# SysCV/sam-pt

Measured on AMD Instinct MI355X. Metric: frames/sec end-to-end (ViT-H + PIPS, 480p, 8 pts, 1 obj) at 1/2/4/8 MI355X, higher is better.
Workload: dtype f16; 1 GPU; SAM vit_h + PIPS, 8 query points, 1 object(s), 24x 480p synthetic frames upscaled to 576x1024, 12 refinement iterations, random-init weights (seed 72); submit=sequential: one blocking SamPt.forward per step, parallelism=sequence-sharded x1, decoder_precision=fp32

## Files before the change

sam_pt_amd/csrc/attention.hip:

```cpp
#include "ops.h"

namespace sampt {

typedef float f32x2 __attribute__((ext_vector_type(2)));

template <typename TQ>
__global__ __launch_bounds__(256) void k_vit_rel_bias(const TQ* __restrict__ qkv, const float* __restrict__ rel_h,
                                                      const float* __restrict__ rel_w, int S, int heads, int hd,
                                                      float* __restrict__ relhT, float* __restrict__ relwT) {
  extern __shared__ float qs[];
  const int qh = blockIdx.x, h = blockIdx.y, b = blockIdx.z;
  const int N = S * S, D = heads * hd, ldq = hd + 1;
  for (int i = threadIdx.x; i < S * hd; i += 256) {
    int t = i / hd, c = i - t * hd;
    qs[t * ldq + c] = (float)qkv[((long)(b * N + qh * S + t)) * 3 * D + h * hd + c];
  }
  __syncthreads();
  const long bh = (long)b * heads + h;
  for (int i = threadIdx.x; i < S * 2 * S; i += 256) {
    int kk = i / S, qw = i - kk * S;
    const float* tab;
    if (kk < S) tab = rel_h + (long)(qh - kk + S - 1) * hd;
    else tab = rel_w + (long)(qw - (kk - S) + S - 1) * hd;
    const float* qv = qs + qw * ldq;
    float a = 0.f;
    for (int c = 0; c < hd; ++c) a += qv[c] * tab[c];
    int q = qh * S + qw;
    if (kk < S) relhT[(bh * S + kk) * N + q] = a;
    else relwT[(bh * S + (kk - S)) * N + q] = a;
  }
}

int vit_rel_bias(const void* qkv, int qkv_f16, const float* rel_h, const float* rel_w, int B, int S, int heads,
                 int hd, float* relh, float* relw, hipStream_t s) {
  dim3 grid(S, heads, B), block(256);
  size_t sh = (size_t)S * (hd + 1) * sizeof(float);
  if (qkv_f16)
    hipLaunchKernelGGL(k_vit_rel_bias<half_t>, grid, block, sh, s, (const half_t*)qkv, rel_h, rel_w, S, heads, hd, relh,
                       relw);
  else
    hipLaunchKernelGGL(k_vit_rel_bias<float>, grid, block, sh, s, (const float*)qkv, rel_h, rel_w, S, heads, hd, relh,
                       relw);
  SAMPT_CHECK_LAUNCH("vit_rel_bias");
  return SAMPT_OK;
}

__global__ __launch_bounds__(256) void k_softmax_rel_rows(float* __restrict__ scores, const float* __restrict__ relhT,
                                                          const float* __restrict__ relwT, int N, int S) {
  __shared__ float red[8];
  const int q = blockIdx.x;
  const long bh = blockIdx.y;
  float* row = scores + (bh * N + q) * N;
  const float* rh = relhT + bh * S * N + q;
  const float* rw = relwT + bh * S * N + q;
  const int tid = threadIdx.x, lane = tid & 63, wave = tid >> 6;
  float m = -INFINITY;
  for (int k = tid; k < N; k += 256) {
    float v = row[k] + rh[(long)(k / S) * N] + rw[(long)(k % S) * N];
    row[k] = v;
    m = fmaxf(m, v);
  }
  m = wave_max(m);
  if (lane == 0) red[wave] = m;
  __syncthreads();
  m = fmaxf(fmaxf(red[0], red[1]), fmaxf(red[2], red[3]));
  float sum = 0.f;
  for (int k = tid; k < N; k += 256) {
    float e = expf(row[k] - m);
    row[k] = e;
    sum += e;
  }
  sum = wave_sum(sum);
  if (lane == 0) red[4 + wave] = sum;
  __syncthreads();
  sum = (red[4] + red[5]) + (red[6] + red[7]);
  for (int k = tid; k < N; k += 256) row[k] = row[k] / sum;
}

int softmax_rel_rows(float* scores, const float* relh, const float* relw, long BH, int Nq, int S, hipStream_t s) {
  if (Nq != S * S) return SAMPT_ERR_ARG;
  hipLaunchKernelGGL(k_softmax_rel_rows, dim3(Nq, (unsigned)BH), dim3(256), 0, s, scores, relh, relw, Nq, S);
  SAMPT_CHECK_LAUNCH("softmax_rel_rows");
  return SAMPT_OK;
}

__device__ half_t g_flash_pad[16] = {(half_t)1.f, (half_t)0.f, (half_t)0.f, (half_t)0.f, (half_t)0.f, (half_t)0.f,
                                     (half_t)0.f, (half_t)0.f, (half_t)0.f, (half_t)0.f, (half_t)0.f, (half_t)0.f,
                                     (half_t)0.f, (half_t)0.f, (half_t)0.f, (half_t)0.f};

template <int HD, int NW, int SG>
__global__ __launch_bounds__(NW * 64, NW == 4 ? 3 : 2) void k_flash_f16(const half_t* __restrict__ qkv, const float* __restrict__ rel_h,
                                                       const float* __restrict__ rel_w, half_t* __restrict__ out, int N,
                                                       int heads, float scale, FlashPad pad, int B, int uh) {
  constexpr int KS = HD / 16;
  constexpr int DT = (HD + 31) / 32;
  constexpr int QT = NW * 32;
  constexpr int NT = NW * 64;
  constexpr bool LROW = DT * 32 > HD;
  constexpr int VP = LROW ? DT * 32 : HD;
  constexpr int RLD = QT + 2;
  constexpr int CPR = HD / 8, CPV = VP / 8;
  constexpr int KSWZ = CPR == 8 ? 7 : (CPR == 4 ? 3 : (CPR == 10 ? 1 : 0)), KSH = CPR == 4 ? 2 : (CPR == 10 ? 3 : 1);
  constexpr int KB = 64 * HD * 2, VB = 64 * VP * 2, RELB = SG * RLD * 2;
  constexpr int BUFB = KB + VB > RELB ? KB + VB : ((RELB + 1023) / 1024) * 1024;
  __shared__ __attribute__((aligned(1024))) char tile_s[BUFB];
  __shared__ half_t relh_s[SG][RLD];
  half_t(*Ks)[64][HD] = (half_t(*)[64][HD])tile_s;
  half_t(*Vs)[64][VP] = (half_t(*)[64][VP])(tile_s + KB);
  half_t(*relw_s)[RLD] = (half_t(*)[RLD])tile_s;
  constexpr int NKI = (CPR + NW - 1) / NW, NVI = (CPV + NW - 1) / NW;
  __shared__ unsigned dma_tab[NKI + NVI][NT];

  const int tid = threadIdx.x, lane = tid & 63, wave = __builtin_amdgcn_readfirstlane(tid >> 6);
  const int li = lane & 31, hi = lane >> 5;
  int bx, h, b;
  flash_wg_decode(blockIdx.x, (N + QT - 1) / QT, heads, B, uh, bx, h, b);
  const int D = heads * HD;
  const long tok0 = (long)b * N;
  const int qblk = bx * QT;
  const int ql = wave * 32 + li;
  const int q = qblk + ql;
  const bool wave_live = qblk + wave * 32 < N;
  constexpr int RPT = SG >= 64 ? 1 : 64 / SG, KTV = SG >= 64 ? 64 : RPT * SG;
  constexpr float LOG2E = 1.4426950408889634f;
  const float c2 = scale * LOG2E;
  const int pw = pad.bias_row ? b % pad.nwin : 0;
  const int pwy = pw / max(pad.nwx, 1), py0 = pwy * SG, px0 = (pw - pwy * max(pad.nwx, 1)) * SG;
  auto is_pad = [&](int t) {
    const int iy = t / SG, ix = t - iy * SG;
    return pad.bias_row != nullptr && (py0 + iy >= pad.gh || px0 + ix >= pad.gw);
  };
  {
    int n = 0;
    for (int i = wave; i < CPR; i += NW, ++n) {
      const int e = i * 64 + lane, slot = e / CPR, c = e - slot * CPR;
      const int sc = min(slot, KTV - 1), siy = sc / SG, six = sc - siy * SG;
      const unsigned off = (unsigned)((c ^ ((slot >> KSH) & KSWZ)) * 16);
      dma_tab[n][tid] = (unsigned)sc | (unsigned)siy << 8 | (pad.bias_row != nullptr && px0 + six >= pad.gw ? 1u << 12 : 0u) | off << 16;
    }
    n = NKI;
    for (int i = wave; i < CPV; i += NW, ++n) {
      const int e = i * 64 + lane, slot = e / CPV, c = e - slot * CPV;
      const int sc = min(slot, KTV - 1), siy = sc / SG, six = sc - siy * SG;
      const int cs = HD == 64 ? c ^ (((slot >> 1) & 1) << 2) : c;
      const unsigned off = (unsigned)(c < CPR ? cs * 16 : (c - CPR) * 16);
      dma_tab[n][tid] = (unsigned)sc | (unsigned)siy << 8 | (pad.bias_row != nullptr && px0 + six >= pad.gw ? 1u << 12 : 0u) |
                        (c < CPR ? 0u : 1u << 13) | off << 16;
    }
  }
  auto dma_tile = [&](int kt0, int kh0, int buf) {
    const half_t* kbase = qkv + tok0 * 3 * D + D + h * HD;
    const unsigned stride = 3u * (unsigned)D * 2u;
    const char* kb = (const char*)kbase;
    const char* vb = (const char*)(kbase + D);
    const char* pk = (const char*)(pad.bias_row ? pad.bias_row + D + h * HD : kbase);
    const char* pv = (const char*)(pad.bias_row ? pad.bias_row + 2 * D + h * HD : kbase);
    int n = 0;
    for (int i = wave; i < CPR; i += NW, ++n) {
      const unsigned t = dma_tab[n][tid];
      const unsigned krow = min((unsigned)kt0 + (t & 255u), (unsigned)(N - 1));
      const int gr = kh0 + (int)(t >> 8 & 15u);
      const bool pd = pad.bias_row != nullptr && ((t & 0x1000u) != 0 || gr >= SG || py0 + gr >= pad.gh);
      const char* src = pd ? pk + (t >> 16) : kb + (__umul24(krow, stride) + (t >> 16));
      __builtin_amdgcn_global_load_lds((const __attribute__((address_space(1))) void*)src,
                                       (__attribute__((address_space(3))) void*)((char*)&Ks[buf][0][0] + i * 1024), 16, 0, 0);
    }
    n = NKI;
    for (int i = wave; i < CPV; i += NW, ++n) {
      const unsigned t = dma_tab[n][tid];
      const unsigned vrow = min((unsigned)kt0 + (t & 255u), (unsigned)(N - 1));
      const int gr = kh0 + (int)(t >> 8 & 15u);
      const bool pd = pad.bias_row != nullptr && ((t & 0x1000u) != 0 || gr >= SG || py0 + gr >= pad.gh);
      const char* src = pd ? pv + (t >> 16) : vb + (__umul24(vrow, stride) + (t >> 16));
      if (LROW && (t & 0x2000u)) src = (const char*)g_flash_pad + (t >> 16);
      __builtin_amdgcn_global_load_lds((const __attribute__((address_space(1))) void*)src,
                                       (__attribute__((address_space(3))) void*)((char*)&Vs[buf][0][0] + i * 1024), 16, 0, 0);
    }
  };

  for (int i = tid; i < SG * RLD; i += NT) {
    (&relh_s[0][0])[i] = (half_t)0.f;
    (&relw_s[0][0])[i] = (half_t)0.f;
  }
  h8 qf[KS];
#pragma unroll
  for (int ks = 0; ks < KS; ++ks) {
    if (q < N && !is_pad(q)) qf[ks] = *(const h8*)(qkv + (tok0 + q) * 3 * D + h * HD + ks * 16 + hi * 8);
    else qf[ks] = (h8){0, 0, 0, 0, 0, 0, 0, 0};
  }
  __syncthreads();
  {
    constexpr int NR = 2 * SG - 1, NTIL = (NR + 31) / 32;
    const int qh = q / SG, qw = q - qh * SG;
#pragma unroll
    for (int tb = 0; tb < 2; ++tb) {
      const float* tab = tb == 0 ? rel_h : rel_w;
      const int qpos = tb == 0 ? qh : qw;
#pragma unroll
      for (int t = 0; t < NTIL; ++t) {
        f32x16 g;
#pragma unroll
        for (int r = 0; r < 16; ++r) g[r] = 0.f;
        const int row = 32 * t + li;
#pragma unroll
        for (int ks = 0; ks < KS; ++ks) {
          h8 tf = (h8){0, 0, 0, 0, 0, 0, 0, 0};
          if (pad.rel_ops) {
            tf = *(const h8*)(pad.rel_ops + ((((long)tb * NTIL + t) * KS + ks) * 64 + lane) * 8);
          } else if (row < NR) {
            const float4* tp = (const float4*)(tab + (long)row * HD + ks * 16 + hi * 8);
            float4 t0 = tp[0], t1 = tp[1];
            tf = (h8){(half_t)t0.x, (half_t)t0.y, (half_t)t0.z, (half_t)t0.w,
                      (half_t)t1.x, (half_t)t1.y, (half_t)t1.z, (half_t)t1.w};
          }
          g = __builtin_amdgcn_mfma_f32_32x32x16_f16(tf, qf[ks], g, 0, 0, 0);
        }
        if (q < N) {
#pragma unroll
          for (int r = 0; r < 16; ++r) {
            const int rho = 32 * t + (r & 3) + 8 * (r >> 2) + 4 * hi;
            const int kx = qpos - rho + SG - 1;
            if (kx >= 0 && kx < SG) {
              if (tb == 0) relh_s[kx][ql] = (half_t)g[r];
              else relw_s[kx][ql] = (half_t)g[r];
            }
          }
        }
      }
    }
  }

  f32x16 o[DT];
#pragma unroll
  for (int dt = 0; dt < DT; ++dt)
#pragma unroll
    for (int r = 0; r < 16; ++r) o[dt][r] = 0.f;
  float m_run = -INFINITY, l_run = 0.f;

  __syncthreads();
  float relw2[32];
#pragma unroll
  for (int kt = 0; kt < 2; ++kt)
#pragma unroll
    for (int r = 0; r < 16; ++r) {
      const int j = kt * 32 + (r & 3) + 8 * (r >> 2) + 4 * hi;
      const int kw = SG >= 64 ? j : j % SG;
      relw2[kt * 16 + r] = j < KTV ? LOG2E * (float)relw_s[kw][ql] : -INFINITY;
    }

  int vl[DT];
  {
    const int s16 = li & 15, r4 = s16 >> 2, cc = s16 & 3, g16 = li >> 4;
#pragma unroll
    for (int dt = 0; dt < DT; ++dt)
      vl[dt] = (4 * hi + r4) * VP * 2 + ((dt * 64 + g16 * 32 + cc * 8) ^ (HD == 64 ? ((r4 >> 1) & 1) << 6 : 0));
  }
  __syncthreads();
  dma_tile(0, 0, 0);
  asm volatile("s_waitcnt vmcnt(0)" ::: "memory");
  __syncthreads();
  for (int kt0 = 0, kh0 = 0, it = 0; kt0 < N; kt0 += KTV, kh0 += RPT, ++it) {
    constexpr int buf = 0;
    if (wave_live) {
    const bool half1 = RPT == 1 || kh0 + 32 / SG < SG;

    f32x16 st[2];
#pragma unroll
    for (int kt = 0; kt < 2; ++kt) {
#pragma unroll
      for (int r = 0; r < 16; ++r) st[kt][r] = 0.f;
      if (kt == 1 && !half1) continue;
#pragma unroll
      for (int ks = 0; ks < KS; ++ks) {
        const int krow = kt * 32 + li;
        h8 kf = *(const h8*)&Ks[buf][krow][((ks * 2 + hi) ^ ((krow >> KSH) & KSWZ)) * 8];
        st[kt] = __builtin_amdgcn_mfma_f32_32x32x16_f16(kf, qf[ks], st[kt], 0, 0, 0);
      }
    }
    float rh[RPT];
#pragma unroll
    for (int jr = 0; jr < RPT; ++jr) rh[jr] = kh0 + jr < SG ? LOG2E * (float)relh_s[kh0 + jr][ql] : -INFINITY;
    float mloc = -INFINITY;
    f32x2 sv2[2][8];
    const f32x2 c2v = (f32x2){c2, c2};
#pragma unroll
    for (int kt = 0; kt < 2; ++kt) {
#pragma unroll
      for (int rp = 0; rp < 8; ++rp) {
        f32x2 x = (f32x2){st[kt][2 * rp], st[kt][2 * rp + 1]};
        x = x * c2v + (f32x2){relw2[kt * 16 + 2 * rp], relw2[kt * 16 + 2 * rp + 1]};
        if (RPT > 1) {
          f32x2 bb;
#pragma unroll
          for (int e = 0; e < 2; ++e) {
            const int r = 2 * rp + e;
            const int j0 = kt * 32 + (r & 3) + 8 * (r >> 2);
            const int ja = min(j0 / SG, RPT - 1), jb = min((j0 + 4) / SG, RPT - 1);
            bb[e] = ja == jb ? rh[ja] : (hi ? rh[jb] : rh[ja]);
          }
          x = x + bb;
        }
        sv2[kt][rp] = x;
        mloc = fmaxf(mloc, fmaxf(x[0], x[1]));
      }
    }
    if (RPT == 1) mloc += rh[0];
    mloc = fmaxf(mloc, __shfl_xor(mloc, 32, 64));
    const float m_new = fmaxf(m_run, mloc);
    const float msub = RPT == 1 ? m_new - rh[0] : m_new;
    const f32x2 mv = (f32x2){msub, msub};
    float lsum = 0.f;
    h8 pb[4];
#pragma unroll
    for (int kt = 0; kt < 2; ++kt) {
      if (kt == 1 && !half1) continue;
#pragma unroll
      for (int r = 0; r < 16; r += 2) {
        const f32x2 e2 = sv2[kt][r >> 1] - mv;
        const float p0 = __builtin_amdgcn_exp2f(e2[0]), p1 = __builtin_amdgcn_exp2f(e2[1]);
        if (!LROW) lsum += p0 + p1;
        f32x2 pp = (f32x2){p0, p1};
        h2 ph = __builtin_convertvector(pp, h2);
        pb[kt * 2 + (r >> 3)][r & 7] = ph[0];
        pb[kt * 2 + (r >> 3)][(r & 7) + 1] = ph[1];
      }
    }
    if (!LROW) lsum += __shfl_xor(lsum, 32, 64);
    if (__any(m_new > m_run)) {
      const float alpha = __builtin_amdgcn_exp2f(m_run - m_new);
      l_run *= alpha;
#pragma unroll
      for (int dt = 0; dt < DT; ++dt)
#pragma unroll
        for (int r = 0; r < 16; ++r) o[dt][r] *= alpha;
      m_run = m_new;
    }
    l_run += lsum;
#pragma unroll
    for (int t = 0; t < 4; ++t) {
      if (t >= 2 && !half1) continue;
#pragma unroll
      for (int dt = 0; dt < DT; ++dt) {
        typedef short s4 __attribute__((ext_vector_type(4)));
        typedef __attribute__((address_space(3))) s4 lds_s4;
        const __attribute__((address_space(3))) char* vb =
            (const __attribute__((address_space(3))) char*)&Vs[buf][0][0] + vl[dt] + 16 * t * VP * 2;
        const s4 v0 = __builtin_amdgcn_ds_read_tr16_b64_v4i16((lds_s4*)vb);
        const s4 v1 = __builtin_amdgcn_ds_read_tr16_b64_v4i16((lds_s4*)(vb + 8 * VP * 2));
        const h8 vf = __builtin_bit_cast(h8, __builtin_shufflevector(v0, v1, 0, 1, 2, 3, 4, 5, 6, 7));
        o[dt] = __builtin_amdgcn_mfma_f32_32x32x16_f16(vf, pb[t], o[dt], 0, 0, 0);
      }
    }
    }
    if (kt0 + KTV < N) {
      __syncthreads();
      dma_tile(kt0 + KTV, kh0 + RPT, 0);
    }
    asm volatile("s_waitcnt vmcnt(0)" ::: "memory");
    __syncthreads();
  }

  if (LROW) {
    constexpr int LR = HD % 32, RL = (LR % 4) + 4 * (LR / 8), HL = (LR / 4) % 2;
    l_run = __shfl(o[DT - 1][RL], li | (HL << 5), 64);
  }
  if (q < N) {
    const float inv = 1.0f / l_run;
    half_t* op = out + (tok0 + q) * D + h * HD;
#pragma unroll
    for (int dt = 0; dt < DT; ++dt) {
#pragma unroll
      for (int g = 0; g < 4; ++g) {
        int d0 = dt * 32 + 8 * g + 4 * hi;
        if (d0 < HD) {
          h4 v = (h4){(half_t)(o[dt][4 * g] * inv), (half_t)(o[dt][4 * g + 1] * inv), (half_t)(o[dt][4 * g + 2] * inv),
                      (half_t)(o[dt][4 * g + 3] * inv)};
          *(h4*)(op + d0) = v;
        }
      }
    }
  }
}

int vit_flash_attention_f16(const half_t* qkv, const float* relh, const float* relw, half_t* out, int B, int S,
                            int heads, int hd, hipStream_t s, FlashPad pad) {
  if (pad.bias_row && (pad.nwx <= 0 || pad.nwin <= 0 || B % pad.nwin)) return SAMPT_ERR_ARG;
  const int N = S * S;
  const float scale = 1.0f / sqrtf((float)hd);
#define FL(HDv, NWv, SGv)                                                                                     \
  hipLaunchKernelGGL((k_flash_f16<HDv, NWv, SGv>), dim3(cdiv(N, NWv * 32) * heads * B), dim3(NWv * 64), 0, s, qkv, relh, relw, \
                     out, N, heads, scale, pad, B, SGv < 64 ? heads : 0)
  if (S == 64 && hd == 80) FL(80, 4, 64);
  else if (S == 64 && hd == 64) FL(64, 4, 64);
  else if (S == 14 && hd == 80) FL(80, 4, 14);
  else if (S == 14 && hd == 64) FL(64, 4, 14);
  else if (S == 16 && hd == 32) FL(32, 4, 16);
  else if (S == 6 && hd == 32) FL(32, 2, 6);
  else return SAMPT_ERR_UNSUPPORTED;
#undef FL
  SAMPT_CHECK_LAUNCH("vit_flash_attention_f16");
  return SAMPT_OK;
}

}
```

Measured before the change: 122.5 frames/s.

## Add double-buffered K ring prefetch to flash attention for small head dims

Adds a RING template variant of the flash attention kernel that double-buffers the K tile and prefetches the next K tile while computing the current one. V loads are issued early and waited on with fine-grained vmcnt counts instead of full barriers. The DMA table also shrinks to 16-bit entries for SG==64. RING is enabled only for the hd=32 shapes (S=16, S=6, likely the PIPS/decoder attention), not the ViT-H hd=80 paths. The m0-based inline asm and the hand-counted waitcnt logic add correctness risk, and the extra K buffer raises LDS use.

After: 122.5 frames/s, median of 2. About the same (-0.0%).

```diff
diff --git a/sam_pt_amd/csrc/attention.hip b/sam_pt_amd/csrc/attention.hip
--- a/sam_pt_amd/csrc/attention.hip
+++ b/sam_pt_amd/csrc/attention.hip
@@ -1,3 +1,5 @@
+#include <type_traits>
+
 #include "ops.h"
 
 namespace sampt {
@@ -88,7 +90,7 @@
                                      (half_t)0.f, (half_t)0.f, (half_t)0.f, (half_t)0.f, (half_t)0.f, (half_t)0.f,
                                      (half_t)0.f, (half_t)0.f, (half_t)0.f, (half_t)0.f};
 
-template <int HD, int NW, int SG>
+template <int HD, int NW, int SG, bool RING>
 __global__ __launch_bounds__(NW * 64, NW == 4 ? 3 : 2) void k_flash_f16(const half_t* __restrict__ qkv, const float* __restrict__ rel_h,
                                                        const float* __restrict__ rel_w, half_t* __restrict__ out, int N,
                                                        int heads, float scale, FlashPad pad, int B, int uh) {
@@ -102,14 +104,25 @@
   constexpr int CPR = HD / 8, CPV = VP / 8;
   constexpr int KSWZ = CPR == 8 ? 7 : (CPR == 4 ? 3 : (CPR == 10 ? 1 : 0)), KSH = CPR == 4 ? 2 : (CPR == 10 ? 3 : 1);
   constexpr int KB = 64 * HD * 2, VB = 64 * VP * 2, RELB = SG * RLD * 2;
-  constexpr int BUFB = KB + VB > RELB ? KB + VB : ((RELB + 1023) / 1024) * 1024;
+  constexpr int RELR = ((RELB + 1023) / 1024) * 1024, K1OFF = KB + VB;
+  constexpr int BUFB = RING ? KB + (VB + KB > RELB ? VB + KB : RELR) : (KB + VB > RELB ? KB + VB : RELR);
   __shared__ __attribute__((aligned(1024))) char tile_s[BUFB];
   __shared__ half_t relh_s[SG][RLD];
-  half_t(*Ks)[64][HD] = (half_t(*)[64][HD])tile_s;
   half_t(*Vs)[64][VP] = (half_t(*)[64][VP])(tile_s + KB);
-  half_t(*relw_s)[RLD] = (half_t(*)[RLD])tile_s;
+  half_t(*relw_s)[RLD] = (half_t(*)[RLD])(RING ? tile_s + KB : tile_s);
+  constexpr bool TAB16 = SG == 64;
+  typedef typename std::conditional<TAB16, unsigned short, unsigned>::type tab_t;
   constexpr int NKI = (CPR + NW - 1) / NW, NVI = (CPV + NW - 1) / NW;
-  __shared__ unsigned dma_tab[NKI + NVI][NT];
+  __shared__ tab_t dma_tab[NKI + NVI][NT];
+  auto tab_pack = [](int slot, int row, bool colpad, bool page, unsigned off) {
+    return TAB16 ? (tab_t)((unsigned)slot | (page ? 1u << 6 : 0u) | (colpad ? 1u << 7 : 0u) | off << 8)
+                 : (tab_t)((unsigned)slot | (unsigned)row << 8 | (colpad ? 1u << 12 : 0u) | (page ? 1u << 13 : 0u) | off << 16);
+  };
+  auto tab_slot = [](unsigned t) { return TAB16 ? t & 63u : t & 255u; };
+  auto tab_row = [](unsigned t) { return TAB16 ? 0 : (int)(t >> 8 & 15u); };
+  auto tab_colpad = [](unsigned t) { return (t & (TAB16 ? 0x80u : 0x1000u)) != 0; };
+  auto tab_page = [](unsigned t) { return (t & (TAB16 ? 0x40u : 0x2000u)) != 0; };
+  auto tab_off = [](unsigned t) { return TAB16 ? t >> 8 : t >> 16; };
 
   const int tid = threadIdx.x, lane = tid & 63, wave = __builtin_amdgcn_readfirstlane(tid >> 6);
   const int li = lane & 31, hi = lane >> 5;
@@ -136,7 +149,7 @@
       const int e = i * 64 + lane, slot = e / CPR, c = e - slot * CPR;
       const int sc = min(slot, KTV - 1), siy = sc / SG, six = sc - siy * SG;
       const unsigned off = (unsigned)((c ^ ((slot >> KSH) & KSWZ)) * 16);
-      dma_tab[n][tid] = (unsigned)sc | (unsigned)siy << 8 | (pad.bias_row != nullptr && px0 + six >= pad.gw ? 1u << 12 : 0u) | off << 16;
+      dma_tab[n][tid] = tab_pack(sc, siy, pad.bias_row != nullptr && px0 + six >= pad.gw, false, off);
     }
     n = NKI;
     for (int i = wave; i < CPV; i += NW, ++n) {
@@ -144,39 +157,57 @@
       const int sc = min(slot, KTV - 1), siy = sc / SG, six = sc - siy * SG;
       const int cs = HD == 64 ? c ^ (((slot >> 1) & 1) << 2) : c;
       const unsigned off = (unsigned)(c < CPR ? cs * 16 : (c - CPR) * 16);
-      dma_tab[n][tid] = (unsigned)sc | (unsigned)siy << 8 | (pad.bias_row != nullptr && px0 + six >= pad.gw ? 1u << 12 : 0u) |
-                        (c < CPR ? 0u : 1u << 13) | off << 16;
-    }
-  }
-  auto dma_tile = [&](int kt0, int kh0, int buf) {
-    const half_t* kbase = qkv + tok0 * 3 * D + D + h * HD;
-    const unsigned stride = 3u * (unsigned)D * 2u;
+      dma_tab[n][tid] = tab_pack(sc, siy, pad.bias_row != nullptr && px0 + six >= pad.gw, c >= CPR, off);
+    }
+  }
+  const half_t* kbase = qkv + tok0 * 3 * D + D + h * HD;
+  const unsigned stride = 3u * (unsigned)D * 2u;
+  auto glds16 = [&](const char* src, char* dst) {
+    if (RING) {
+      unsigned keep;
+      const unsigned lds_dst = (unsigned)(size_t)(__attribute__((address_space(3))) char*)dst;
+      asm volatile("s_mov_b32 %0, m0\n\ts_mov_b32 m0, %2\n\ts_nop 0\n\tglobal_load_lds_dwordx4 %1, off\n\ts_mov_b32 m0, %0"
+                   : "=&s"(keep)
+                   : "v"(src), "s"(lds_dst)
+                   : "memory");
+    } else {
+      __builtin_amdgcn_global_load_lds((const __attribute__((address_space(1))) void*)src,
+                                       (__attribute__((address_space(3))) void*)dst, 16, 0, 0);
+    }
+  };
+  auto dma_k = [&](int kt0, int kh0, int koff) {
     const char* kb = (const char*)kbase;
-    const char* vb = (const char*)(kbase + D);
     const char* pk = (const char*)(pad.bias_row ? pad.bias_row + D + h * HD : kbase);
-    const char* pv = (const char*)(pad.bias_row ? pad.bias_row + 2 * D + h * HD : kbase);
     int n = 0;
     for (int i = wave; i < CPR; i += NW, ++n) {
       const unsigned t = dma_tab[n][tid];
-      const unsigned krow = min((unsigned)kt0 + (t & 255u), (unsigned)(N - 1));
-      const int gr = kh0 + (int)(t >> 8 & 15u);
-      const bool pd = pad.bias_row != nullptr && ((t & 0x1000u) != 0 || gr >= SG || py0 + gr >= pad.gh);
-      const char* src = pd ? pk + (t >> 16) : kb + (__umul24(krow, stride) + (t >> 16));
-      __builtin_amdgcn_global_load_lds((const __attribute__((address_space(1))) void*)src,
-                                       (__attribute__((address_space(3))) void*)((char*)&Ks[buf][0][0] + i * 1024), 16, 0, 0);
-    }
-    n = NKI;
+      const unsigned krow = min((unsigned)kt0 + tab_slot(t), (unsigned)(N - 1));
+      const int gr = kh0 + tab_row(t);
+      const bool pd = pad.bias_row != nullptr && (tab_colpad(t) || gr >= SG || py0 + gr >= pad.gh);
+      const char* src = pd ? pk + tab_off(t) : kb + (__umul24(krow, stride) + tab_off(t));
+      glds16(src, tile_s + koff + i * 1024);
+    }
+  };
+  auto dma_v = [&](int kt0, int kh0) {
+    const char* vb = (const char*)(kbase + D);
+    const char* pv = (const char*)(pad.bias_row ? pad.bias_row + 2 * D + h * HD : kbase);
+    int n = NKI;
     for (int i = wave; i < CPV; i += NW, ++n) {
       const unsigned t = dma_tab[n][tid];
-      const unsigned vrow = min((unsigned)kt0 + (t & 255u), (unsigned)(N - 1));
-      const int gr = kh0 + (int)(t >> 8 & 15u);
-      const bool pd = pad.bias_row != nullptr && ((t & 0x1000u) != 0 || gr >= SG || py0 + gr >= pad.gh);
-      const char* src = pd ? pv + (t >> 16) : vb + (__umul24(vrow, stride) + (t >> 16));
-      if (LROW && (t & 0x2000u)) src = (const char*)g_flash_pad + (t >> 16);
-      __builtin_amdgcn_global_load_lds((const __attribute__((address_space(1))) void*)src,
-                                       (__attribute__((address_space(3))) void*)((char*)&Vs[buf][0][0] + i * 1024), 16, 0, 0);
-    }
-  };
+      const unsigned vrow = min((unsigned)kt0 + tab_slot(t), (unsigned)(N - 1));
+      const int gr = kh0 + tab_row(t);
+      const bool pd = pad.bias_row != nullptr && (tab_colpad(t) || gr >= SG || py0 + gr >= pad.gh);
+      const char* src = pd ? pv + tab_off(t) : vb + (__umul24(vrow, stride) + tab_off(t));
+      if (LROW && tab_page(t)) src = (const char*)g_flash_pad + tab_off(t);
+      glds16(src, (char*)&Vs[0][0][0] + i * 1024);
+    }
+  };
+  auto lds_barrier = [&]() {
+    asm volatile("s_waitcnt lgkmcnt(0)" ::: "memory");
+    __builtin_amdgcn_s_barrier();
+    asm volatile("" ::: "memory");
+  };
+  if (RING) dma_k(0, 0, 0);
 
   for (int i = tid; i < SG * RLD; i += NT) {
     (&relh_s[0][0])[i] = (half_t)0.f;
@@ -188,7 +219,8 @@
     if (q < N && !is_pad(q)) qf[ks] = *(const h8*)(qkv + (tok0 + q) * 3 * D + h * HD + ks * 16 + hi * 8);
     else qf[ks] = (h8){0, 0, 0, 0, 0, 0, 0, 0};
   }
-  __syncthreads();
+  if (RING) lds_barrier();
+  else __syncthreads();
   {
     constexpr int NR = 2 * SG - 1, NTIL = (NR + 31) / 32;
     const int qh = q / SG, qw = q - qh * SG;
@@ -237,7 +269,8 @@
     for (int r = 0; r < 16; ++r) o[dt][r] = 0.f;
   float m_run = -INFINITY, l_run = 0.f;
 
-  __syncthreads();
+  if (RING) lds_barrier();
+  else __syncthreads();
   float relw2[32];
 #pragma unroll
   for (int kt = 0; kt < 2; ++kt)
@@ -255,12 +288,31 @@
     for (int dt = 0; dt < DT; ++dt)
       vl[dt] = (4 * hi + r4) * VP * 2 + ((dt * 64 + g16 * 32 + cc * 8) ^ (HD == 64 ? ((r4 >> 1) & 1) << 6 : 0));
   }
-  __syncthreads();
-  dma_tile(0, 0, 0);
-  asm volatile("s_waitcnt vmcnt(0)" ::: "memory");
-  __syncthreads();
+  if (!RING) {
+    __syncthreads();
+    dma_k(0, 0, 0), dma_v(0, 0);
+    asm volatile("s_waitcnt vmcnt(0)" ::: "memory");
+    __syncthreads();
+  }
+  constexpr int NKF = CPR / NW;
+  static_assert(NKF >= 1 && NKI <= 3, "vmcnt of step 5");
+  const bool k_short = NKF != NKI && wave >= CPR % NW;
+  auto wait_v = [&](bool k_behind) {
+    if (!k_behind) asm volatile("s_waitcnt vmcnt(0) lgkmcnt(0)" ::: "memory");
+    else if (k_short) asm volatile("s_waitcnt vmcnt(%0) lgkmcnt(0)" ::"n"(NKF) : "memory");
+    else asm volatile("s_waitcnt vmcnt(%0) lgkmcnt(0)" ::"n"(NKI) : "memory");
+  };
   for (int kt0 = 0, kh0 = 0, it = 0; kt0 < N; kt0 += KTV, kh0 += RPT, ++it) {
-    constexpr int buf = 0;
+    const int koff = RING && (it & 1) ? K1OFF : 0;
+    const half_t(*Kt)[HD] = (const half_t(*)[HD])(tile_s + koff);
+    if (RING) {
+      asm volatile("s_waitcnt vmcnt(0)" ::: "memory");
+      lds_barrier();
+      dma_v(kt0, kh0);
+      __builtin_amdgcn_sched_barrier(0);
+      if (kt0 + KTV < N) dma_k(kt0 + KTV, kh0 + RPT, koff ^ K1OFF);
+      __builtin_amdgcn_sched_barrier(0);
+    }
     if (wave_live) {
     const bool half1 = RPT == 1 || kh0 + 32 / SG < SG;
 
@@ -273,7 +325,8 @@
 #pragma unroll
       for (int ks = 0; ks < KS; ++ks) {
         const int krow = kt * 32 + li;
-        h8 kf = *(const h8*)&Ks[buf][krow][((ks * 2 + hi) ^ ((krow >> KSH) & KSWZ)) * 8];
+        const int kc = KSWZ == 1 ? ks * 2 + (hi ^ ((krow >> KSH) & 1)) : (ks * 2 + hi) ^ ((krow >> KSH) & KSWZ);
+        h8 kf = *(const h8*)&Kt[krow][kc * 8];
         st[kt] = __builtin_amdgcn_mfma_f32_32x32x16_f16(kf, qf[ks], st[kt], 0, 0, 0);
       }
     }
@@ -336,6 +389,13 @@
       m_run = m_new;
     }
     l_run += lsum;
+    if (RING) {
+      asm volatile("" ::"v"(pb[0]), "v"(pb[1]));
+      if (half1) asm volatile("" ::"v"(pb[2]), "v"(pb[3]));
+      wait_v(kt0 + KTV < N);
+      __builtin_amdgcn_s_barrier();
+      asm volatile("" ::: "memory");
+    }
 #pragma unroll
     for (int t = 0; t < 4; ++t) {
       if (t >= 2 && !half1) continue;
@@ -344,20 +404,26 @@
         typedef short s4 __attribute__((ext_vector_type(4)));
         typedef __attribute__((address_space(3))) s4 lds_s4;
         const __attribute__((address_space(3))) char* vb =
-            (const __attribute__((address_space(3))) char*)&Vs[buf][0][0] + vl[dt] + 16 * t * VP * 2;
+            (const __attribute__((address_space(3))) char*)&Vs[0][0][0] + vl[dt] + 16 * t * VP * 2;
         const s4 v0 = __builtin_amdgcn_ds_read_tr16_b64_v4i16((lds_s4*)vb);
         const s4 v1 = __builtin_amdgcn_ds_read_tr16_b64_v4i16((lds_s4*)(vb + 8 * VP * 2));
         const h8 vf = __builtin_bit_cast(h8, __builtin_shufflevector(v0, v1, 0, 1, 2, 3, 4, 5, 6, 7));
         o[dt] = __builtin_amdgcn_mfma_f32_32x32x16_f16(vf, pb[t], o[dt], 0, 0, 0);
       }
     }
-    }
-    if (kt0 + KTV < N) {
+    } else if (RING) {
+      wait_v(kt0 + KTV < N);
+      __builtin_amdgcn_s_barrier();
+      asm volatile("" ::: "memory");
+    }
+    if (!RING) {
+      if (kt0 + KTV < N) {
+        __syncthreads();
+        dma_k(kt0 + KTV, kh0 + RPT, 0), dma_v(kt0 + KTV, kh0 + RPT);
+      }
+      asm volatile("s_waitcnt vmcnt(0)" ::: "memory");
       __syncthreads();
-      dma_tile(kt0 + KTV, kh0 + RPT, 0);
-    }
-    asm volatile("s_waitcnt vmcnt(0)" ::: "memory");
-    __syncthreads();
+    }
   }
 
   if (LROW) {
@@ -387,15 +453,15 @@
   if (pad.bias_row && (pad.nwx <= 0 || pad.nwin <= 0 || B % pad.nwin)) return SAMPT_ERR_ARG;
   const int N = S * S;
   const float scale = 1.0f / sqrtf((float)hd);
-#define FL(HDv, NWv, SGv)                                                                                     \
-  hipLaunchKernelGGL((k_flash_f16<HDv, NWv, SGv>), dim3(cdiv(N, NWv * 32) * heads * B), dim3(NWv * 64), 0, s, qkv, relh, relw, \
+#define FL(HDv, NWv, SGv, RGv)                                                                                   \
+  hipLaunchKernelGGL((k_flash_f16<HDv, NWv, SGv, RGv>), dim3(cdiv(N, NWv * 32) * heads * B), dim3(NWv * 64), 0, s, qkv, relh, relw, \
                      out, N, heads, scale, pad, B, SGv < 64 ? heads : 0)
-  if (S == 64 && hd == 80) FL(80, 4, 64);
-  else if (S == 64 && hd == 64) FL(64, 4, 64);
-  else if (S == 14 && hd == 80) FL(80, 4, 14);
-  else if (S == 14 && hd == 64) FL(64, 4, 14);
-  else if (S == 16 && hd == 32) FL(32, 4, 16);
-  else if (S == 6 && hd == 32) FL(32, 2, 6);
+  if (S == 64 && hd == 80) FL(80, 4, 64, false);
+  else if (S == 64 && hd == 64) FL(64, 4, 64, false);
+  else if (S == 14 && hd == 80) FL(80, 4, 14, false);
+  else if (S == 14 && hd == 64) FL(64, 4, 14, false);
+  else if (S == 16 && hd == 32) FL(32, 4, 16, true);
+  else if (S == 6 && hd == 32) FL(32, 2, 6, true);
   else return SAMPT_ERR_UNSUPPORTED;
 #undef FL
   SAMPT_CHECK_LAUNCH("vit_flash_attention_f16");
```
